# FFTAI/Wiki-GRx-Gym

Hardware: AMD Instinct MI355X
Metric: env-steps/sec GR1T1 rough-terrain @4096 envs (higher is better)
Workload: dtype f32

## Files before the change

include/grx_ppo.h:

```cpp
#ifndef GRX_PPO_H
#define GRX_PPO_H
#ifdef __cplusplus
extern "C" {
#endif

int grx_ppo_loss_partials_size(int batch);

int grx_ppo_loss(int batch, int num_actions, const float* mu, const float* std, const float* value,
                 const float* actions, const float* old_logp, const float* old_mu, const float* old_sigma,
                 const float* advantages, const float* returns, const float* target_values,
                 float clip_param, float value_loss_coef, float entropy_coef, int use_clipped_value_loss,
                 float* out, float* d_mu, float* d_std, float* d_value, float* partials, void* stream);

int grx_ppo_colsum_partials_size(int rows, int cols);
int grx_ppo_colsum(int rows, int cols, const float* x, float* out, float* partials, void* stream);

int grx_ppo_elu_backward_colsum(int rows, int cols, const float* dy, const float* y, float* dz, float* out, float* partials, void* stream);

int grx_ppo_store_transition(int N, int num_obs, int num_pri, int num_actions,
                             const float* obs, const float* pri, const float* actions, const float* mu, const float* sigma,
                             const float* values, const float* logp, const float* rewards, const unsigned char* dones,
                             const unsigned char* time_outs, float gamma,
                             float* st_obs, float* st_pri, float* st_actions, float* st_mu, float* st_sigma, float* st_values,
                             float* st_logp, float* st_rewards, unsigned char* st_dones,
// ... 2 lines not shown
#define GRX_PPO_TAIL_MAX 24
typedef struct grx_ppo_tail_tensors {
    int n, pad;
    float* param[GRX_PPO_TAIL_MAX]; const float* grad[GRX_PPO_TAIL_MAX]; float* exp_avg[GRX_PPO_TAIL_MAX]; float* exp_avg_sq[GRX_PPO_TAIL_MAX];
    float* step[GRX_PPO_TAIL_MAX];
    long long numel[GRX_PPO_TAIL_MAX];
} grx_ppo_tail_tensors;
typedef struct grx_ppo_tail_args {
    const float* loss;
    const float* bad_flag;
    const float* kl;
    float* lr;
    const float *value_loss, *surrogate_loss;
    float* sums;
    float* partials;
    int adaptive, pad;
    float desired_kl, lr_min, lr_max, max_grad_norm;
    double beta1, beta2, eps;
} grx_ppo_tail_args;
int grx_ppo_step_tail_blocks(const grx_ppo_tail_tensors* t);
int grx_ppo_step_tail(const grx_ppo_tail_tensors* t, const grx_ppo_tail_args* a, void* stream);

#define GRX_PPO_GATHER_MAX 12
int grx_ppo_gather_rows(int n_tensors, const float* const* src, float* const* dst, const int* widths, const long long* idx, int mb, void* stream);

int grx_mlp_layer(int M, int K, int N, const float* X, const float* W, const float* bias, float* Y, int elu, void* stream);

int grx_mlp_layer_bf16(int M, int K, int N, const float* X, const float* W, const float* bias, float* Y, int elu, void* stream);
int grx_mlp_input_grad_bf16(int M, int N, int K, const float* dZ, const float* W, float* dX, void* stream);
int grx_mlp_weight_grad_bf16_partials_size(int M, int N, int K);
int grx_mlp_weight_grad_bf16(int M, int N, int K, const float* dZ, const float* X, float* dW, float* partials, void* stream);

int grx_mlp_policy_head(int M, int K, int A, const float* X, const float* W, const float* bias, const float* std,
                        const float* eps, float* actions, float* logp, float* mu, float* sigma, void* stream);

int grx_obs_norm_partials_size(int rows, int cols);
int grx_obs_norm_moments(int rows, int cols, const float* x, float* partials, void* stream);
int grx_obs_norm_merge(int n_partials, int cols, int stride, const float* partials, long long* count, float* mean, float* var, float* std,
                       void* stream);
int grx_obs_norm_combine(int n_partials, int cols, const float* partials, float* out, void* stream);
int grx_obs_norm_apply(int rows, int cols, const float* x, const float* mean, const float* std, float eps, float* y, void* stream);
int grx_obs_norm_step(int rows, int cols, const float* x, float* partials, long long* count, float* mean, float* var, float* std, float eps,
                      float* y, void* stream);

int grx_obs_history_push(int N, int D, int H, const float* obs, const unsigned char* dones, int fill_all, const float* src, float* dst,
                         void* stream);

int grx_distill_loss_partials_size(int batch, int A);
int grx_distill_loss(int batch, int A, const float* student_mu, const float* teacher_mu, int huber, float* out, float* d_mu, float* partials,
                     void* stream);
int grx_distill_store(int N, int D, int A, const float* obs, const float* labels, const float* rewards, const unsigned char* dones,
                      float* st_obs, float* st_labels, unsigned char* st_dones,
                      float* cur_rew, float* cur_len, float* done_rew, float* done_len, void* stream);

int grx_lstm_cell(int M, int D, int H, const float* x, const float* h_prev, const float* c_prev, const unsigned char* reset,
                  const float* W_ih, const float* W_hh, const float* b_ih, const float* b_hh, float* h, float* c, float* acts, void* stream);
int grx_lstm_cell_preact(int M, int D, int H, const float* x, const float* h_prev, const unsigned char* reset, const float* W_ih,
                         const float* W_hh, const float* b_ih, const float* b_hh, float* G, void* stream);
int grx_lstm_cell_backward(int M, int H, const float* dh, const float* dc_in, const float* acts, const float* c_prev,
                           const unsigned char* reset, float* dG, float* dc_prev, void* stream);

#define GRX_SYM_MAX_WIDTH 2048
int grx_sym_gather_rows(int n_tensors, const float* const* src, float* const* dst, const int* widths, const int* modes,
                        const int* const* perm, const float* const* scale, const float* const* offset, const long long* idx, int mb,
                        void* stream);

int grx_rnd_reward_partials_size(int N);
int grx_rnd_reward(int N, int E, const float* pred, const float* targ, float gamma, float weight, float eps, float* ret, long long* count,
                   float* mean, float* var, float* std, float* rewards, float* intrinsic, float* raw, float* partials, void* stream);

#ifdef __cplusplus
}
#endif

#include "grx_ppo_noise.h"
#include "grx_ppo_smooth.h"
#include "grx_ppo_est.h"
#include "grx_ppo_gae.h"
#include "grx_ppo_gp.h"
#include "grx_ppo_ln.h"
#include "grx_ppo_mc.h"
#include "grx_ppo_beta.h"
#include "grx_ppo_cenet.h"
#endif
```

wiki-grx-gym_amd/csrc/grx_ppo.hip:

```cpp
#include <hip/hip_runtime.h>
#include <stdint.h>
#include "../../include/grx_ppo.h"

namespace {
constexpr int MAXA = 32;
constexpr int NTHR = 256;
constexpr int NRED = 3 + MAXA;

__device__ inline float nmax(float a, float b) { return (a > b || a != a) ? a : b; }
__device__ inline float nmin(float a, float b) { return (a < b || a != a) ? a : b; }

__device__ inline double wave_sum(double v) {
#pragma unroll
    for (int o = 32; o > 0; o >>= 1) v += __shfl_down(v, o);
    return v;
}

template <int A>
__global__ __launch_bounds__(NTHR) void ppo_loss_kernel(int B, const float* __restrict__ mu, const float* __restrict__ stdp,
                                                         const float* __restrict__ value, const float* __restrict__ actions,
                                                         const float* __restrict__ old_logp, const float* __restrict__ old_mu,
                                                         const float* __restrict__ old_sigma, const float* __restrict__ adv_,
                                                         const float* __restrict__ ret_, const float* __restrict__ tv_,
                                                         float clip, float vcoef, int use_clipped,
// ... 21 lines not shown
        const float rc = nmin(nmax(ratio, lo), hi);
        const float s1 = -adv * ratio, s2 = -adv * rc;
        const float surr = nmax(s1, s2);
        const float w1 = s1 > s2 ? 1.f : (s1 == s2 ? 0.5f : 0.f), w2 = 1.f - w1;
        const float in_range = (ratio >= lo && ratio <= hi) ? 1.f : 0.f;
        const float g_ratio = -adv * (w1 + w2 * in_range);
        const float g_logp = g_ratio * ratio * invB;
#pragma unroll
        for (int k = 0; k < A; ++k) {
            const float s = sg[k], inv2 = 1.0f / (s * s);
            const float half = 0.5f * inv2;
            const float np = 0.f * (g_logp * (((df[k] * df[k] * half) * half) * 2.0f * (2.0f * s)) - g_logp / s);
            d_mu[(size_t)i * A + k] = g_logp * df[k] * inv2 + np;
            red[3 + k] = g_logp * (df[k] * df[k] * inv2 / s - 1.0f / s) + np;
        }
        const float v = value[i], ret = ret_[i];
        float vl, gv;
        if (use_clipped) {
            const float tv = tv_[i];
            const float dv = v - tv;
            const float vc = tv + nmin(nmax(dv, -clip), clip);
            const float l1 = (v - ret) * (v - ret), l2 = (vc - ret) * (vc - ret);
            vl = nmax(l1, l2);
            const float u1 = l1 > l2 ? 1.f : (l1 == l2 ? 0.5f : 0.f), u2 = 1.f - u1;
            const float vin = (dv >= -clip && dv <= clip) ? 1.f : 0.f;
            gv = u1 * 2.0f * (v - ret) + (vin != 0.f ? u2 * 2.0f * (vc - ret) : 0.f);
        } else {
            vl = (ret - v) * (ret - v);
            gv = -2.0f * (ret - v);
        }
        d_value[i] = vcoef * gv * invB;
        red[0] = surr; red[1] = vl; red[2] = kl;
    }
    __shared__ double s_red[NTHR / 64][3 + A];
    const int lane = threadIdx.x & 63, wv = threadIdx.x >> 6;
#pragma unroll
    for (int k = 0; k < 3 + A; ++k) {
        const double t = wave_sum((double)red[k]);
        if (lane == 0) s_red[wv][k] = t;
    }
    __syncthreads();
    if (threadIdx.x < 3 + A) {
        double t = 0.0;
#pragma unroll
        for (int w = 0; w < NTHR / 64; ++w) t += s_red[w][threadIdx.x];
        partials[(size_t)blockIdx.x * NRED + threadIdx.x] = t;
    }
}

__global__ __launch_bounds__(64) void ppo_loss_finalize(int B, int A, int nblk, const double* __restrict__ partials,
                                                         const float* __restrict__ stdp, float vcoef, float ecoef,
                                                         float* __restrict__ out, float* __restrict__ d_std) {
    const int k = threadIdx.x;
    double t = 0.0;
    constexpr int STAGE = 4096;
    __shared__ double s_p[STAGE];
    const bool staged = nblk * NRED <= STAGE;
    if (staged) {
        for (int i = k; i < nblk * NRED; i += 64) s_p[i] = partials[i];
        __syncthreads();
    }
    if (k < 3 + A)
        for (int b = 0; b < nblk; ++b) t += staged ? s_p[b * NRED + k] : partials[(size_t)b * NRED + k];
    __shared__ double s_t[64];
    s_t[k] = t;
    __syncthreads();
    if (k >= 3 && k < 3 + A) d_std[k - 3] = (float)t - ecoef / stdp[k - 3];
    if (k == 0) {
        const float surr = (float)(s_t[0] / (double)B), vl = (float)(s_t[1] / (double)B), klm = (float)(s_t[2] / (double)B);
        float ent = 0.f;
        for (int a = 0; a < A; ++a) ent += 1.4189385332046727f + logf(stdp[a]);
        out[0] = surr; out[1] = vl; out[2] = surr + vcoef * vl - ecoef * ent; out[3] = klm;
    }
}

template <int A>
void launch(int nblk, hipStream_t st, int B, const float* mu, const float* stdp, const float* value, const float* actions,
            const float* old_logp, const float* old_mu, const float* old_sigma, const float* adv, const float* ret, const float* tv,
            float clip, float vcoef, int use_clipped, float* d_mu, float* d_value, double* partials) {
    hipLaunchKernelGGL(ppo_loss_kernel<A>, dim3(nblk), dim3(NTHR), 0, st, B, mu, stdp, value, actions, old_logp, old_mu, old_sigma,
                       adv, ret, tv, clip, vcoef, use_clipped, d_mu, d_value, partials);
}

constexpr int CS_ROWS = 256;
__global__ __launch_bounds__(256) void colsum_partial(int rows, int cols, const float* __restrict__ x, float* __restrict__ partials) {
    const int lane = threadIdx.x & 63, wv = threadIdx.x >> 6;
    const int col = blockIdx.x * 64 + lane;
    const int r0 = blockIdx.y * CS_ROWS, r1 = min(rows, r0 + CS_ROWS);
    float acc = 0.f;
    if (col < cols) {
        float a0 = 0.f, a1 = 0.f, a2 = 0.f, a3 = 0.f;
        int r = r0 + wv;
        for (; r + 12 < r1; r += 16) {
            a0 += x[(size_t)r * cols + col]; a1 += x[(size_t)(r + 4) * cols + col];
            a2 += x[(size_t)(r + 8) * cols + col]; a3 += x[(size_t)(r + 12) * cols + col];
        }
        for (; r < r1; r += 4) a0 += x[(size_t)r * cols + col];
        acc = (a0 + a1) + (a2 + a3);
    }
    __shared__ float s_acc[4][64];
    s_acc[wv][lane] = acc;
    __syncthreads();
    if (wv == 0 && col < cols) partials[(size_t)blockIdx.y * cols + col] = (s_acc[0][lane] + s_acc[1][lane]) + (s_acc[2][lane] + s_acc[3][lane]);
}
__global__ __launch_bounds__(256) void elu_bwd_colsum_partial(int rows, int cols, const float* __restrict__ dy, const float* __restrict__ y,
                                                              float* __restrict__ dz, float* __restrict__ partials) {
    const int lane = threadIdx.x & 63, wv = threadIdx.x >> 6;
    const int col = blockIdx.x * 64 + lane;
    const int r0 = blockIdx.y * CS_ROWS, r1 = min(rows, r0 + CS_ROWS);
    float acc = 0.f;
    if (col < cols) {
        float a0 = 0.f, a1 = 0.f, a2 = 0.f, a3 = 0.f;
        auto one = [&](const int r) -> float {
            const size_t o = (size_t)r * cols + col;
            const float yy = y[o];
            const float g = dy[o] * (yy > 0.f ? 1.0f : yy + 1.0f);
            dz[o] = g;
            return g;
        };
        int r = r0 + wv;
        for (; r + 12 < r1; r += 16) { a0 += one(r); a1 += one(r + 4); a2 += one(r + 8); a3 += one(r + 12); }
        for (; r < r1; r += 4) a0 += one(r);
        acc = (a0 + a1) + (a2 + a3);
    }
    __shared__ float s_acc[4][64];
    s_acc[wv][lane] = acc;
    __syncthreads();
    if (wv == 0 && col < cols) partials[(size_t)blockIdx.y * cols + col] = (s_acc[0][lane] + s_acc[1][lane]) + (s_acc[2][lane] + s_acc[3][lane]);
}
__global__ __launch_bounds__(256) void colsum_final(int cols, int nslab, const float* __restrict__ partials, float* __restrict__ out) {
    const int lane = threadIdx.x & 63, col = blockIdx.x * 4 + (threadIdx.x >> 6);
    if (col >= cols) return;
    float t = 0.f;
    for (int b = lane; b < nslab; b += 64) t += partials[(size_t)b * cols + col];
#pragma unroll
    for (int o = 32; o > 0; o >>= 1) t += __shfl_down(t, o);
    if (lane == 0) out[col] = t;
}

typedef float f32x16 __attribute__((ext_vector_type(16)));
constexpr int ML_BM = 64, ML_BN = 64, ML_KC = 64, ML_LD = 65;

__device__ inline float elu1(float x) { return x > 0.f ? x : expm1f(x); }

template <bool VEC>
__device__ inline void ml_fetch(const float* __restrict__ G, int rows, int ld, int r0, int k0, int tid, float4 v[4]) {
    const int kq = k0 + 4 * (tid & 15);
#pragma unroll
    for (int p = 0; p < 4; ++p) {
        const int r = r0 + 16 * p + (tid >> 4);
        const float* g = G + (size_t)min(r, rows - 1) * ld + kq;
        float4 x = {0.f, 0.f, 0.f, 0.f};
        if (r < rows) {
            if (VEC) { if (kq < ld) x = *reinterpret_cast<const float4*>(g); }
            else { if (kq < ld) x.x = g[0]; if (kq + 1 < ld) x.y = g[1]; if (kq + 2 < ld) x.z = g[2]; if (kq + 3 < ld) x.w = g[3]; }
        }
        v[p] = x;
    }
}
__device__ inline void ml_stash(float* __restrict__ S, int tid, const float4 v[4]) {
    const int kq = 4 * (tid & 15);
#pragma unroll
    for (int p = 0; p < 4; ++p) {
        float* s = S + kq * ML_LD + 16 * p + (tid >> 4);
        s[0] = v[p].x; s[ML_LD] = v[p].y; s[2 * ML_LD] = v[p].z; s[3 * ML_LD] = v[p].w;
    }
}

struct HeadOut { const float* stdp; const float* eps; float* actions; float* logp; float* mu; float* sigma; };
template <bool ELU, bool VEC, bool HEAD = false>
__global__ __launch_bounds__(256) void mlp_layer_kernel(int M, int K, int N, const float* __restrict__ X, const float* __restrict__ W,
                                                         const float* __restrict__ bias, float* __restrict__ Y, HeadOut ho = HeadOut()) {
#if defined(__HIP_DEVICE_COMPILE__) && !defined(__gfx950__)
#error "mlp_layer_kernel keeps 65 KB of static LDS: gfx950 (160 KB per CU) only -- this library is built for MI355X, see the Makefile"
#endif
    __shared__ float Xs[2][ML_KC * ML_LD], Ws[2][ML_KC * ML_LD];
    const int tid = threadIdx.x, lane = tid & 63, wv = tid >> 6, wy = wv >> 1, wx = wv & 1;
    const int m0 = blockIdx.x * ML_BM, n0 = blockIdx.y * ML_BN;
    float4 xr[4], wr[4];
    f32x16 acc;
#pragma unroll
    for (int r = 0; r < 16; ++r) acc[r] = 0.f;
    ml_fetch<VEC>(X, M, K, m0, 0, tid, xr);
    ml_fetch<VEC>(W, N, K, n0, 0, tid, wr);
    ml_stash(Xs[0], tid, xr); ml_stash(Ws[0], tid, wr);
    __syncthreads();
    int buf = 0;
    for (int k0 = 0; k0 < K; k0 += ML_KC, buf ^= 1) {
        const bool more = k0 + ML_KC < K;
        if (more) { ml_fetch<VEC>(X, M, K, m0, k0 + ML_KC, tid, xr); ml_fetch<VEC>(W, N, K, n0, k0 + ML_KC, tid, wr); }
        const float* xa = Xs[buf] + (lane >> 5) * ML_LD + 32 * wy + (lane & 31);
        const float* wb = Ws[buf] + (lane >> 5) * ML_LD + 32 * wx + (lane & 31);
        const int nk = min(ML_KC, K - k0);
        if (nk == ML_KC) {
            float av[ML_KC / 2], bv[ML_KC / 2];
#pragma unroll
            for (int kk = 0; kk < ML_KC / 2; ++kk) { av[kk] = xa[2 * kk * ML_LD]; bv[kk] = wb[2 * kk * ML_LD]; }
#pragma unroll
            for (int kk = 0; kk < ML_KC / 2; ++kk) acc = __builtin_amdgcn_mfma_f32_32x32x2f32(av[kk], bv[kk], acc, 0, 0, 0);
        } else {
            for (int kk = 0; kk < (nk + 1) / 2; ++kk)
                acc = __builtin_amdgcn_mfma_f32_32x32x2f32(xa[2 * kk * ML_LD], wb[2 * kk * ML_LD], acc, 0, 0, 0);
        }
        if (more) { ml_stash(Xs[buf ^ 1], tid, xr); ml_stash(Ws[buf ^ 1], tid, wr); }
        __syncthreads();
// ... 294 lines not shown
```

wiki-grx-gym_amd/rl/fused_loss.py:

```python
import ctypes as C
import os

import torch

_LIB = None


def load_ppo_library():
    global _LIB
    if _LIB is None:
        path = os.environ.get("GRX_PPO_LIB") or os.path.join(os.path.dirname(os.path.dirname(os.path.abspath(__file__))), "csrc", "libgrx_ppo.so")
        if not os.path.exists(path):
            raise RuntimeError(f"{path} is missing: build it with `python -c 'import __graft_entry__ as g; g.build()'` "
                               "(there is no silent fallback for CUDA tensors; set GRX_PPO_FUSED_LOSS=0 to use the torch expression)")
        lib = C.CDLL(path)
        fp = C.c_void_p
        lib.grx_ppo_loss.restype = C.c_int
        lib.grx_ppo_loss.argtypes = [C.c_int, C.c_int] + [fp] * 10 + [C.c_float, C.c_float, C.c_float, C.c_int] + [fp] * 5 + [C.c_void_p]
        lib.grx_ppo_loss_partials_size.restype = C.c_int
        lib.grx_ppo_loss_partials_size.argtypes = [C.c_int]
        lib.grx_ppo_colsum.restype = C.c_int
        lib.grx_ppo_colsum.argtypes = [C.c_int, C.c_int, fp, fp, fp, C.c_void_p]
        lib.grx_ppo_colsum_partials_size.restype = C.c_int
        lib.grx_ppo_colsum_partials_size.argtypes = [C.c_int, C.c_int]
# ... 3 lines not shown
        lib.grx_ppo_elu_backward_colsum.argtypes = [C.c_int, C.c_int, fp, fp, fp, fp, fp, C.c_void_p]
        lib.grx_ppo_gather_rows.restype = C.c_int
        lib.grx_ppo_gather_rows.argtypes = [C.c_int, C.POINTER(C.c_void_p), C.POINTER(C.c_void_p), C.POINTER(C.c_int), fp, C.c_int, C.c_void_p]
        lib.grx_mlp_layer.restype = C.c_int
        lib.grx_mlp_layer.argtypes = [C.c_int] * 3 + [fp] * 4 + [C.c_int, C.c_void_p]
        lib.grx_mlp_layer_bf16.restype = C.c_int
        lib.grx_mlp_layer_bf16.argtypes = [C.c_int] * 3 + [fp] * 4 + [C.c_int, C.c_void_p]
        lib.grx_mlp_input_grad_bf16.restype = C.c_int
        lib.grx_mlp_input_grad_bf16.argtypes = [C.c_int] * 3 + [fp] * 3 + [C.c_void_p]
        lib.grx_mlp_weight_grad_bf16_partials_size.restype = C.c_int
        lib.grx_mlp_weight_grad_bf16_partials_size.argtypes = [C.c_int] * 3
        lib.grx_mlp_weight_grad_bf16.restype = C.c_int
        lib.grx_mlp_weight_grad_bf16.argtypes = [C.c_int] * 3 + [fp] * 4 + [C.c_void_p]
        lib.grx_mlp_policy_head.restype = C.c_int
        lib.grx_mlp_policy_head.argtypes = [C.c_int] * 3 + [fp] * 9 + [C.c_void_p]
        lib.grx_ppo_step_tail.restype = C.c_int
        lib.grx_ppo_step_tail.argtypes = [C.c_void_p, C.c_void_p, C.c_void_p]
        lib.grx_ppo_step_tail_blocks.restype = C.c_int
        lib.grx_ppo_step_tail_blocks.argtypes = [C.c_void_p]
        lib.grx_obs_norm_partials_size.restype = C.c_int
        lib.grx_obs_norm_partials_size.argtypes = [C.c_int, C.c_int]
        lib.grx_obs_norm_moments.restype = C.c_int
        lib.grx_obs_norm_moments.argtypes = [C.c_int, C.c_int, fp, fp, C.c_void_p]
        lib.grx_obs_norm_merge.restype = C.c_int
        lib.grx_obs_norm_merge.argtypes = [C.c_int, C.c_int, C.c_int] + [fp] * 5 + [C.c_void_p]
        lib.grx_obs_norm_combine.restype = C.c_int
        lib.grx_obs_norm_combine.argtypes = [C.c_int, C.c_int, fp, fp, C.c_void_p]
        lib.grx_obs_norm_apply.restype = C.c_int
        lib.grx_obs_norm_apply.argtypes = [C.c_int, C.c_int, fp, fp, fp, C.c_float, fp, C.c_void_p]
        lib.grx_obs_norm_step.restype = C.c_int
        lib.grx_obs_norm_step.argtypes = [C.c_int, C.c_int] + [fp] * 6 + [C.c_float, fp, C.c_void_p]
        lib.grx_obs_history_push.restype = C.c_int
        lib.grx_obs_history_push.argtypes = [C.c_int] * 3 + [fp, fp, C.c_int, fp, fp, C.c_void_p]
        lib.grx_distill_loss_partials_size.restype = C.c_int
        lib.grx_distill_loss_partials_size.argtypes = [C.c_int, C.c_int]
        lib.grx_distill_loss.restype = C.c_int
        lib.grx_distill_loss.argtypes = [C.c_int, C.c_int, fp, fp, C.c_int, fp, fp, fp, C.c_void_p]
        lib.grx_distill_store.restype = C.c_int
        lib.grx_distill_store.argtypes = [C.c_int] * 3 + [fp] * 11 + [C.c_void_p]
        pp = C.POINTER(C.c_void_p)
        lib.grx_sym_gather_rows.restype = C.c_int
        lib.grx_sym_gather_rows.argtypes = [C.c_int, pp, pp, C.POINTER(C.c_int), C.POINTER(C.c_int), pp, pp, pp, fp, C.c_int, C.c_void_p]
        lib.grx_rnd_reward_partials_size.restype = C.c_int
        lib.grx_rnd_reward_partials_size.argtypes = [C.c_int]
        lib.grx_rnd_reward.restype = C.c_int
        lib.grx_rnd_reward.argtypes = [C.c_int, C.c_int, fp, fp, C.c_float, C.c_float, C.c_float] + [fp] * 9 + [C.c_void_p]
        lib.grx_ppo_loss_sd_partials_size.restype = C.c_int
        lib.grx_ppo_loss_sd_partials_size.argtypes = [C.c_int]
        lib.grx_ppo_loss_sd.restype = C.c_int
        lib.grx_ppo_loss_sd.argtypes = [C.c_int, C.c_int, fp, C.c_int] + [fp] * 8 + [C.c_float, C.c_float, C.c_float, C.c_int] + [fp] * 4 + [C.c_void_p]
        lib.grx_mlp_policy_head_sd.restype = C.c_int
        lib.grx_mlp_policy_head_sd.argtypes = [C.c_int] * 3 + [fp] * 3 + [C.c_int] + [fp] * 5 + [C.c_void_p]
        lib.grx_smooth_gather_rows.restype = C.c_int
        lib.grx_smooth_gather_rows.argtypes = ([C.c_int, pp, pp, C.POINTER(C.c_int), fp, C.c_int, C.c_int, C.c_int, fp, C.c_int, C.c_int, fp,
                                                C.c_float, fp, C.c_void_p])
        lib.grx_smooth_loss_partials_size.restype = C.c_int
        lib.grx_smooth_loss_partials_size.argtypes = [C.c_int, C.c_int]
        lib.grx_smooth_loss.restype = C.c_int
        lib.grx_smooth_loss.argtypes = [C.c_int, C.c_int, fp, C.c_int, C.c_int, fp, C.c_float, C.c_float, fp, fp, fp, C.c_void_p]
        lib.grx_est_forward.restype = C.c_int
        lib.grx_est_forward.argtypes = [fp, C.c_int, C.c_int, fp, C.c_int, fp, C.POINTER(C.c_int), fp, fp, C.c_void_p]
        lib.grx_gae_partials_size.restype = C.c_int
        lib.grx_gae_partials_size.argtypes = [C.c_int, C.c_int]
        lib.grx_gae_returns.restype = C.c_int
        lib.grx_gae_returns.argtypes = [C.c_int, C.c_int] + [fp] * 4 + [C.c_float] * 3 + [fp] * 10 + [C.c_void_p]
        lib.grx_gp_seed.restype = C.c_int
        lib.grx_gp_seed.argtypes = [C.c_int, C.c_int] + [fp] * 4 + [C.c_void_p]
        lib.grx_gp_gate.restype = C.c_int
        lib.grx_gp_gate.argtypes = [C.c_int, C.c_int] + [fp] * 3 + [C.c_void_p]
        lib.grx_gp_sqnorm_partials_size.restype = C.c_int
        lib.grx_gp_sqnorm_partials_size.argtypes = [C.c_int, C.c_int]
        lib.grx_gp_sqnorm.restype = C.c_int
        lib.grx_gp_sqnorm.argtypes = [C.c_int, C.c_int] + [fp] * 3 + [C.c_void_p]
        lib.grx_gp_gate_backward.restype = C.c_int
        lib.grx_gp_gate_backward.argtypes = [C.c_int, C.c_int] + [fp] * 8 + [C.c_void_p]
        lib.grx_gp_seed_backward.restype = C.c_int
        lib.grx_gp_seed_backward.argtypes = [C.c_int, C.c_int] + [fp] * 8 + [C.c_void_p]
        lib.grx_ln_elu_forward.restype = C.c_int
        lib.grx_ln_elu_forward.argtypes = [C.c_int, C.c_int, fp, fp, fp, C.c_float, fp, fp, fp, C.c_void_p]
        lib.grx_ln_elu_backward_partials_size.restype = C.c_int
        lib.grx_ln_elu_backward_partials_size.argtypes = [C.c_int, C.c_int]
        lib.grx_ln_elu_backward.restype = C.c_int
        lib.grx_ln_elu_backward.argtypes = [C.c_int, C.c_int] + [fp] * 11 + [C.c_void_p]
        _LIB = lib
    return _LIB


TAIL_MAX = 24


class _TailTensors(C.Structure):
    _fields_ = [("n", C.c_int), ("pad", C.c_int), ("param", C.c_void_p * TAIL_MAX), ("grad", C.c_void_p * TAIL_MAX),
                ("exp_avg", C.c_void_p * TAIL_MAX), ("exp_avg_sq", C.c_void_p * TAIL_MAX), ("step", C.c_void_p * TAIL_MAX),
                ("numel", C.c_longlong * TAIL_MAX)]


class _TailArgs(C.Structure):
    _fields_ = [("loss", C.c_void_p), ("bad_flag", C.c_void_p), ("kl", C.c_void_p), ("lr", C.c_void_p), ("value_loss", C.c_void_p),
                ("surrogate_loss", C.c_void_p), ("sums", C.c_void_p), ("partials", C.c_void_p), ("adaptive", C.c_int), ("pad", C.c_int),
                ("desired_kl", C.c_float), ("lr_min", C.c_float), ("lr_max", C.c_float), ("max_grad_norm", C.c_float),
                ("beta1", C.c_double), ("beta2", C.c_double), ("eps", C.c_double)]


class StepTail:

    @staticmethod
    def supported(optimizer, params):
        g = optimizer.param_groups
        return (len(g) == 1 and len(params) <= TAIL_MAX and not g[0].get("amsgrad") and not g[0].get("maximize") and g[0].get("weight_decay", 0) == 0
                and all(p.is_cuda and p.dtype == torch.float32 and p.is_contiguous() for p in params))

    def __init__(self, optimizer, params, lr_t):
        self.lib = load_ppo_library()
        self.opt, self.params, self.lr_t = optimizer, list(params), lr_t
        self.t, self.a = _TailTensors(), _TailArgs()
        self.key, self.partials = None, None

    def _state(self, p):
        st = self.opt.state[p]
        if "exp_avg" not in st:
            st["step"] = torch.zeros((), dtype=torch.float32, device=p.device)
            st["exp_avg"] = torch.zeros_like(p, memory_format=torch.preserve_format)
            st["exp_avg_sq"] = torch.zeros_like(p, memory_format=torch.preserve_format)
        return st

    def __call__(self, loss, kl, value_loss, surrogate_loss, sums, adaptive, desired_kl, lr_min, lr_max, max_grad_norm, bad_flag=None):
        t, a = self.t, self.a
        sts = [self._state(p) for p in self.params]
        key = tuple(x.data_ptr() for p, st in zip(self.params, sts) for x in (p, st["exp_avg"], st["exp_avg_sq"], st["step"]))
        if key != self.key:
            t.n = len(self.params)
            for i, (p, st) in enumerate(zip(self.params, sts)):
                if not (st["step"].is_cuda and st["step"].dtype == torch.float32 and st["exp_avg"].is_contiguous() and st["exp_avg_sq"].is_contiguous()):
                    raise RuntimeError("StepTail: the optimizer state is not torch's fused / capturable layout")
                t.param[i], t.exp_avg[i], t.exp_avg_sq[i], t.step[i], t.numel[i] = p.data_ptr(), st["exp_avg"].data_ptr(), st["exp_avg_sq"].data_ptr(), st["step"].data_ptr(), p.numel()
            nb = self.lib.grx_ppo_step_tail_blocks(C.byref(t))
            if nb < 1:
                raise RuntimeError("grx_ppo_step_tail_blocks failed")
            self.partials = torch.empty(nb, device=self.params[0].device, dtype=torch.float32)
            self.key = key
        for i, p in enumerate(self.params):
            g = p.grad
            if g is None or not g.is_contiguous() or g.dtype != torch.float32:
                raise RuntimeError("StepTail: every parameter needs a contiguous fp32 .grad")
            t.grad[i] = g.data_ptr()
        g0 = self.opt.param_groups[0]
        a.loss, a.kl, a.lr = loss.data_ptr(), kl.data_ptr(), self.lr_t.data_ptr()
        a.bad_flag = bad_flag.data_ptr() if bad_flag is not None else None
        a.value_loss, a.surrogate_loss = value_loss.data_ptr(), surrogate_loss.data_ptr()
        a.sums = sums.data_ptr() if sums is not None else None
        a.partials = self.partials.data_ptr()
        a.adaptive = int(bool(adaptive))
        a.desired_kl, a.lr_min, a.lr_max, a.max_grad_norm = float(desired_kl or 0.0), float(lr_min), float(lr_max), float(max_grad_norm)
        a.beta1, a.beta2, a.eps = float(g0["betas"][0]), float(g0["betas"][1]), float(g0["eps"])
        dev = self.params[0].device
        with torch.cuda.device(dev):
            rc = self.lib.grx_ppo_step_tail(C.byref(t), C.byref(a), C.c_void_p(torch.cuda.current_stream(dev).cuda_stream))
        if rc != 0:
            raise RuntimeError(f"grx_ppo_step_tail failed ({rc})")


def _f32c(x):
    return x if (x.dtype == torch.float32 and x.is_contiguous()) else x.contiguous().float()


class FusedPPOLoss(torch.autograd.Function):
# ... 22 lines not shown
        return out

    @staticmethod
    def backward(ctx, g):
        d_mu, d_std, d_value = ctx.saved_tensors
        gl = g[2]
        return (d_mu * gl, d_std * gl, (d_value * gl).reshape(ctx.value_shape)) + (None,) * 11


def fused_ppo_loss(mu, std, value, actions, old_logp, old_mu, old_sigma, advantages, returns, target_values,
                   clip_param, value_loss_coef, entropy_coef, use_clipped_value_loss):
    return FusedPPOLoss.apply(mu, std, value, actions, old_logp, old_mu, old_sigma, advantages, returns, target_values,
                              clip_param, value_loss_coef, entropy_coef, use_clipped_value_loss)


class FusedPPOLossSD(torch.autograd.Function):

    @staticmethod
    def forward(ctx, raw, value, actions, old_logp, old_mu, old_sigma, advantages, returns, target_values,
                log_std, clip_param, value_loss_coef, entropy_coef, use_clipped_value_loss):
        lib = load_ppo_library()
        B, A = actions.shape
        if tuple(raw.shape) != (B, 2 * A):
            raise RuntimeError(f"fused_ppo_loss_sd: raw is {tuple(raw.shape)}, expected {(B, 2 * A)} ([mean | s] of {A} actions)")
        raw_c, value_c = _f32c(raw), _f32c(value).reshape(-1)
        data = [_f32c(t) for t in (actions, old_logp, old_mu, old_sigma, advantages, returns, target_values)]
        out = torch.empty(4, device=raw.device, dtype=torch.float32)
        d_raw = torch.empty_like(raw_c)
        d_value = torch.empty_like(value_c)
        partials = torch.empty(lib.grx_ppo_loss_sd_partials_size(B), device=raw.device, dtype=torch.float32)
        stream = torch.cuda.current_stream(raw.device).cuda_stream
        with torch.cuda.device(raw.device):
            rc = lib.grx_ppo_loss_sd(B, A, raw_c.data_ptr(), int(bool(log_std)), value_c.data_ptr(), *[t.data_ptr() for t in data],
                                     float(clip_param), float(value_loss_coef), float(entropy_coef), int(bool(use_clipped_value_loss)),
                                     out.data_ptr(), d_raw.data_ptr(), d_value.data_ptr(), partials.data_ptr(), C.c_void_p(stream))
        if rc != 0:
            raise RuntimeError(f"grx_ppo_loss_sd failed ({rc}): batch {B}, num_actions {A}")
        ctx.save_for_backward(d_raw, d_value)
        ctx.value_shape = value.shape
        return out

    @staticmethod
    def backward(ctx, g):
        d_raw, d_value = ctx.saved_tensors
        gl = g[2]
        return (d_raw * gl, (d_value * gl).reshape(ctx.value_shape)) + (None,) * 12


def fused_ppo_loss_sd(raw, value, actions, old_logp, old_mu, old_sigma, advantages, returns, target_values,
                      log_std, clip_param, value_loss_coef, entropy_coef, use_clipped_value_loss):
    return FusedPPOLossSD.apply(raw, value, actions, old_logp, old_mu, old_sigma, advantages, returns, target_values,
                                log_std, clip_param, value_loss_coef, entropy_coef, use_clipped_value_loss)


def colsum(x):
    lib = load_ppo_library()
    x = _f32c(x)
    rows, cols = x.shape
    out = torch.empty(cols, device=x.device, dtype=torch.float32)
    partials = torch.empty(lib.grx_ppo_colsum_partials_size(rows, cols), device=x.device, dtype=torch.float32)
    with torch.cuda.device(x.device):
        rc = lib.grx_ppo_colsum(rows, cols, x.data_ptr(), out.data_ptr(), partials.data_ptr(),
                                C.c_void_p(torch.cuda.current_stream(x.device).cuda_stream))
    if rc != 0:
        raise RuntimeError(f"grx_ppo_colsum failed ({rc}): {rows} x {cols}")
    return out


def elu_backward_colsum(dy, y):
    lib = load_ppo_library()
    dy, y = _f32c(dy), _f32c(y)
    rows, cols = dy.shape
    dz = torch.empty_like(dy)
    out = torch.empty(cols, device=dy.device, dtype=torch.float32)
    partials = torch.empty(lib.grx_ppo_colsum_partials_size(rows, cols), device=dy.device, dtype=torch.float32)
    with torch.cuda.device(dy.device):
        rc = lib.grx_ppo_elu_backward_colsum(rows, cols, dy.data_ptr(), y.data_ptr(), dz.data_ptr(), out.data_ptr(), partials.data_ptr(),
                                             C.c_void_p(torch.cuda.current_stream(dy.device).cuda_stream))
    if rc != 0:
        raise RuntimeError(f"grx_ppo_elu_backward_colsum failed ({rc}): {rows} x {cols}")
    return dz, out


def store_transition(storage, step, obs, pri, actions, mu, sigma, values, logp, rewards, dones, time_outs, gamma, log=None):
    lib = load_ppo_library()
    N = storage.num_envs
    ptr = lambda t: t.data_ptr() if t is not None else None
    for t in (obs, pri, actions, mu, sigma, values, logp, rewards):
        if t is not None and not (t.is_cuda and t.dtype == torch.float32 and t.is_contiguous()):
            raise RuntimeError("store_transition needs contiguous float32 CUDA tensors")
    def as_u8(t):
        if t.dtype == torch.bool:
            t = t.view(torch.uint8)
        elif t.dtype != torch.uint8:
            t = (t != 0).to(torch.uint8)
        if not (t.is_cuda and t.is_contiguous() and t.numel() == N):
            raise RuntimeError("store_transition needs contiguous CUDA dones / time_outs with one entry per env")
        return t
    d8 = as_u8(dones)
    t8 = None if time_outs is None else as_u8(time_outs)
    sp = storage.pri_observations
    lg = log if log is not None else (None, None, None, None)
    with torch.cuda.device(obs.device):
        rc = lib.grx_ppo_store_transition(
            N, obs.shape[1], pri.shape[1] if (pri is not None and sp is not None) else 0, actions.shape[1],
            ptr(obs), ptr(pri) if sp is not None else None, ptr(actions), ptr(mu), ptr(sigma), ptr(values), ptr(logp), ptr(rewards), ptr(d8), ptr(t8),
            float(gamma), ptr(storage.observations[step]), ptr(sp[step]) if sp is not None else None, ptr(storage.actions[step]), ptr(storage.mu[step]),
            ptr(storage.sigma[step]), ptr(storage.values[step]), ptr(storage.actions_log_prob[step]), ptr(storage.rewards[step]), ptr(storage.dones[step]),
            ptr(lg[0]), ptr(lg[1]), ptr(lg[2]), ptr(lg[3]), C.c_void_p(torch.cuda.current_stream(obs.device).cuda_stream))
    if rc != 0:
        raise RuntimeError(f"grx_ppo_store_transition failed ({rc})")


def _linears_of(mlp):
    mods = list(mlp.model)
    lin = []
    for i, m in enumerate(mods):
        if i % 2 == 0:
            if not isinstance(m, torch.nn.Linear):
                return None
            lin.append((m.weight, m.bias))
        elif not (isinstance(m, torch.nn.ELU) and m.alpha == 1.0):
            return None
    return lin if len(mods) % 2 == 1 else None


LN_MAX_COLS = 1024


def ln_fused():
    return os.environ.get("GRX_LN_FUSED", "1") != "0"


def _layers_of(mlp):
    mods = list(mlp.model)
    layers, i = [], 0
    while i < len(mods):
        m = mods[i]
        if not isinstance(m, torch.nn.Linear):
            return None
        if i + 1 == len(mods):
            layers.append((m.weight, m.bias, None))
            return layers
        norm = None
        if isinstance(mods[i + 1], torch.nn.LayerNorm):
            norm = mods[i + 1]
            if not (norm.elementwise_affine and norm.bias is not None and tuple(norm.normalized_shape) == (m.out_features,)
                    and m.out_features <= LN_MAX_COLS):
                return None
            i += 1
        if not (i + 1 < len(mods) and isinstance(mods[i + 1], torch.nn.ELU) and mods[i + 1].alpha == 1.0):
            return None
        layers.append((m.weight, m.bias, norm))
        i += 2
    return None


def mlp_can_fuse(mlp, x):
    if not (x.is_cuda and x.dtype == torch.float32 and x.dim() == 2):
        return False
    layers = _layers_of(mlp)
    return layers is not None and (ln_fused() or all(n is None for _, _, n in layers))


def ln_elu_forward(z, gamma, beta, eps, stats=True):
    lib = load_ppo_library()
# ... 208 lines not shown
```

wiki-grx-gym_amd/rl/modules.py:

```python
import torch
import torch.nn as nn
from torch.distributions import Normal

PRECISIONS = ("fp32", "bf16")
_ACTIVATIONS = {"elu": nn.ELU, "selu": nn.SELU, "relu": nn.ReLU, "crelu": nn.ReLU, "lrelu": nn.LeakyReLU,
                "tanh": nn.Tanh, "sigmoid": nn.Sigmoid}


def get_activation(name):
    if name not in _ACTIVATIONS:
        print("invalid activation function!")
        return None
    return _ACTIVATIONS[name]()


import os

_FUSED_ELU_FORWARD = os.environ.get("GRX_PPO_FUSED_FWD", "1") != "0"
_FUSED_ELU_BACKWARD = os.environ.get("GRX_PPO_FUSED_ELU", "1") != "0"
_TRAIN_LINEAR = os.environ.get("GRX_PPO_LINEAR", "colsum")


class _TrainLinear(torch.autograd.Function):

    @staticmethod
    def _blas(pin):
        prev = torch.backends.cuda.preferred_blas_library()
        if pin:
            torch.backends.cuda.preferred_blas_library("cublaslt")
        return prev

    @staticmethod
    def forward(ctx, x, weight, bias):
        prev = _TrainLinear._blas(weight.shape[0] == 1)
        try:
            y = torch.addmm(bias, x, weight.t())
        finally:
            torch.backends.cuda.preferred_blas_library(prev)
        ctx.save_for_backward(x, weight)
        return y

    @staticmethod
    def backward(ctx, dy):
        from .fused_loss import colsum
        x, weight = ctx.saved_tensors
        prev = _TrainLinear._blas(weight.shape[0] == 1)
        try:
            dx = dy @ weight if ctx.needs_input_grad[0] else None
            return dx, dy.t() @ x, colsum(dy)
        finally:
            torch.backends.cuda.preferred_blas_library(prev)


class _TrainLinearELU(torch.autograd.Function):

    @staticmethod
    def forward(ctx, x, weight, bias, bf16):
        ctx.bf16 = bf16
        if bf16:
            from .fused_loss import linear_elu
            y = linear_elu(x, weight, bias, bf16=True)
        elif _FUSED_ELU_FORWARD and x.is_contiguous() and weight.is_contiguous():
            from .fused_loss import linear_elu
            y = linear_elu(x, weight, bias)
        else:
            prev = _TrainLinear._blas(weight.shape[0] == 1)
            try:
                y = torch.nn.functional.elu(torch.addmm(bias, x, weight.t()))
            finally:
                torch.backends.cuda.preferred_blas_library(prev)
        ctx.save_for_backward(x, weight, y)
        return y

    @staticmethod
    def backward(ctx, dy):
        from .fused_loss import elu_backward_colsum
        x, weight, y = ctx.saved_tensors
        dz, db = elu_backward_colsum(dy, y)
        if ctx.bf16:
            from .fused_loss import input_grad_bf16, weight_grad_bf16
            dx = input_grad_bf16(dz, weight) if ctx.needs_input_grad[0] else None
            return dx, weight_grad_bf16(dz, x), db, None
        prev = _TrainLinear._blas(weight.shape[0] == 1)
        try:
            dx = dz @ weight if ctx.needs_input_grad[0] else None
            return dx, dz.t() @ x, db, None
        finally:
            torch.backends.cuda.preferred_blas_library(prev)


def ln_elu_torch(x, weight, bias, gamma, beta, eps):
    z = torch.addmm(bias, x, weight.t())
    return torch.nn.functional.elu(torch.nn.functional.layer_norm(z, (z.shape[-1],), gamma, beta, eps)), z


def ln_elu_backward_torch(dy, y, z, gamma, eps):
    m = z.mean(-1, keepdim=True)
    d = z - m
    s = 1.0 / torch.sqrt((d * d).mean(-1, keepdim=True) + eps)
    xh = d * s
    g = dy * torch.where(y > 0, torch.ones_like(y), y + 1.0)
    q = g * gamma
    c1, c2 = q.mean(-1, keepdim=True), (q * xh).mean(-1, keepdim=True)
    dz = s * ((q - c1) - xh * c2)
    return dz, (g * xh).sum(0), g.sum(0), dz.sum(0)


class _TrainLinearLNELU(torch.autograd.Function):

    @staticmethod
    def forward(ctx, x, weight, bias, gamma, beta, eps):
        from .fused_loss import ln_fused
        ctx.eps, ctx.fused = float(eps), bool(x.is_cuda and ln_fused())
        if ctx.fused:
            from .fused_loss import _f32c, _layer, ln_elu_forward, load_ppo_library
            with torch.cuda.device(x.device):
                z = _layer(load_ppo_library(), _f32c(x), _f32c(weight), bias, False, torch.cuda.current_stream(x.device).cuda_stream)
            y, mean, rstd = ln_elu_forward(z, gamma, beta, ctx.eps)
            ctx.save_for_backward(x, weight, gamma, z, y, mean, rstd)
            return y
        prev = _TrainLinear._blas(x.is_cuda and weight.shape[0] == 1)
        try:
            y, z = ln_elu_torch(x, weight, bias, gamma, beta, ctx.eps)
        finally:
            torch.backends.cuda.preferred_blas_library(prev)
        ctx.save_for_backward(x, weight, gamma, z, y)
        return y

    @staticmethod
    def backward(ctx, dy):
        if ctx.fused:
            from .fused_loss import ln_elu_backward
            x, weight, gamma, z, y, mean, rstd = ctx.saved_tensors
            dz, dgamma, dbeta, db = ln_elu_backward(dy, y, z, mean, rstd, gamma)
        else:
            x, weight, gamma, z, y = ctx.saved_tensors
            dz, dgamma, dbeta, db = ln_elu_backward_torch(dy, y, z, gamma, ctx.eps)
        prev = _TrainLinear._blas(x.is_cuda and weight.shape[0] == 1)
        try:
            dx = dz @ weight if ctx.needs_input_grad[0] else None
            return dx, dz.t() @ x, db, dgamma, dbeta, None
        finally:
            torch.backends.cuda.preferred_blas_library(prev)


class MLP(nn.Module):
    def __init__(self, input_size, output_size, hidden_dims=(256, 256, 256), activation="relu", layer_norm=False, layer_norm_eps=1e-5, **_):
        super().__init__()
        self.input_size, self.output_size, self.hidden_dims = input_size, output_size, list(hidden_dims)
        self.layer_norm, self.layer_norm_eps = bool(layer_norm), float(layer_norm_eps)
        if self.layer_norm and activation != "elu":
            raise ValueError(f"MLP: layer_norm=True needs activation='elu' (the fused LayerNorm + ELU pass), not {activation!r}")
        if self.layer_norm and not self.layer_norm_eps > 0.0:
            raise ValueError(f"MLP: layer_norm_eps must be above 0, not {layer_norm_eps!r}")
        if self.layer_norm and any(not 1 <= int(h) <= 1024 for h in hidden_dims):
            raise ValueError(f"MLP: layer_norm=True covers hidden widths of 1..1024 (include/grx_ppo_ln.h), not {list(hidden_dims)}")
        dims = [input_size] + list(hidden_dims)
        layers = []
        for a, b in zip(dims[:-1], dims[1:]):
            if self.layer_norm:
# ... 273 lines not shown
```

Measured before the change: 97.81 million.

## Add fused f32 MFMA hidden-layer backward computing dX and split-K dW in one kernel

Adds a hidden-layer backward path for fp32 ELU layers. It runs the ELU-grad column sum, then one persistent MFMA kernel that computes both the input gradient and split-K partial weight gradients from a shared work list, then a finish kernel that reduces the dW and bias partials. It replaces separate BLAS GEMMs plus the colsum, and is enabled only for shape/batch ranges listed in a hand-tuned table. The kernel is gfx950-only and needs an extra partials buffer allocation on every call.

```diff
diff --git a/include/grx_ppo.h b/include/grx_ppo.h
--- a/include/grx_ppo.h
+++ b/include/grx_ppo.h
@@ -108,4 +108,5 @@
 #include "grx_ppo_mc.h"
 #include "grx_ppo_beta.h"
 #include "grx_ppo_cenet.h"
+#include "grx_ppo_bwd.h"
 #endif
diff --git a/include/grx_ppo_bwd.h b/include/grx_ppo_bwd.h
--- /dev/null
+++ b/include/grx_ppo_bwd.h
@@ -0,0 +1,20 @@
+#ifndef GRX_PPO_BWD_H
+#define GRX_PPO_BWD_H
+#ifdef __cplusplus
+extern "C" {
+#endif
+
+int grx_mlp_hidden_backward_f32_partials_size(int M, int N, int K);
+
+int grx_mlp_hidden_backward_f32(int M, int N, int K,
+                                const float* dY, const float* Y,
+                                const float* X, const float* W,
+                                float* dZ,
+                                float* dX,
+                                float* dW, float* db,
+                                float* partials, void* stream);
+
+#ifdef __cplusplus
+}
+#endif
+#endif
diff --git a/wiki-grx-gym_amd/csrc/grx_ppo.hip b/wiki-grx-gym_amd/csrc/grx_ppo.hip
--- a/wiki-grx-gym_amd/csrc/grx_ppo.hip
+++ b/wiki-grx-gym_amd/csrc/grx_ppo.hip
@@ -127,7 +127,7 @@
                        adv, ret, tv, clip, vcoef, use_clipped, d_mu, d_value, partials);
 }
 
-constexpr int CS_ROWS = 256;
+#include "grx_ppo_colsum.h"
 __global__ __launch_bounds__(256) void colsum_partial(int rows, int cols, const float* __restrict__ x, float* __restrict__ partials) {
     const int lane = threadIdx.x & 63, wv = threadIdx.x >> 6;
     const int col = blockIdx.x * 64 + lane;
@@ -141,31 +141,6 @@
             a2 += x[(size_t)(r + 8) * cols + col]; a3 += x[(size_t)(r + 12) * cols + col];
         }
         for (; r < r1; r += 4) a0 += x[(size_t)r * cols + col];
-        acc = (a0 + a1) + (a2 + a3);
-    }
-    __shared__ float s_acc[4][64];
-    s_acc[wv][lane] = acc;
-    __syncthreads();
-    if (wv == 0 && col < cols) partials[(size_t)blockIdx.y * cols + col] = (s_acc[0][lane] + s_acc[1][lane]) + (s_acc[2][lane] + s_acc[3][lane]);
-}
-__global__ __launch_bounds__(256) void elu_bwd_colsum_partial(int rows, int cols, const float* __restrict__ dy, const float* __restrict__ y,
-                                                              float* __restrict__ dz, float* __restrict__ partials) {
-    const int lane = threadIdx.x & 63, wv = threadIdx.x >> 6;
-    const int col = blockIdx.x * 64 + lane;
-    const int r0 = blockIdx.y * CS_ROWS, r1 = min(rows, r0 + CS_ROWS);
-    float acc = 0.f;
-    if (col < cols) {
-        float a0 = 0.f, a1 = 0.f, a2 = 0.f, a3 = 0.f;
-        auto one = [&](const int r) -> float {
-            const size_t o = (size_t)r * cols + col;
-            const float yy = y[o];
-            const float g = dy[o] * (yy > 0.f ? 1.0f : yy + 1.0f);
-            dz[o] = g;
-            return g;
-        };
-        int r = r0 + wv;
-        for (; r + 12 < r1; r += 16) { a0 += one(r); a1 += one(r + 4); a2 += one(r + 8); a3 += one(r + 12); }
-        for (; r < r1; r += 4) a0 += one(r);
         acc = (a0 + a1) + (a2 + a3);
     }
     __shared__ float s_acc[4][64];
diff --git a/wiki-grx-gym_amd/csrc/grx_ppo_bwd.hip b/wiki-grx-gym_amd/csrc/grx_ppo_bwd.hip
--- /dev/null
+++ b/wiki-grx-gym_amd/csrc/grx_ppo_bwd.hip
@@ -0,0 +1,231 @@
+#include <hip/hip_runtime.h>
+#include <stdint.h>
+#include "../../include/grx_ppo.h"
+
+namespace {
+#include "grx_ppo_colsum.h"
+
+typedef float f32x16 __attribute__((ext_vector_type(16)));
+constexpr int PT = 128, PKC = 32, PLD = PT + 4, NT = 256;
+constexpr int SLOTS = 512;
+constexpr int MIN_SLAB = 128;
+
+struct Plan {
+    int M, N, K;
+    int tkx, ndx;
+    int tkw, tw, slab, nslab;
+    int nitems;
+};
+
+inline int cdiv(int a, int b) { return (a + b - 1) / b; }
+
+inline Plan make_plan(int M, int N, int K, bool dx) {
+    Plan p;
+    p.M = M; p.N = N; p.K = K;
+    p.tkx = cdiv(K, PT);
+    p.ndx = dx ? cdiv(M, PT) * p.tkx : 0;
+    p.tkw = cdiv(K, PT);
+    p.tw = cdiv(N, PT) * p.tkw;
+    int slab = cdiv(N, PKC) * PKC;
+    if (slab > 512) slab = 512;
+    while (slab > MIN_SLAB && (long long)cdiv(M, slab) * p.tw < 2 * SLOTS) slab = cdiv(slab / 2, PKC) * PKC;
+    if (slab < MIN_SLAB) slab = MIN_SLAB;
+    p.slab = slab;
+    p.nslab = cdiv(M, slab);
+    p.nitems = p.ndx + p.nslab * p.tw;
+    return p;
+}
+
+struct Walk { int a, step, b, lim_a, lim_b; };
+template <bool VEC>
+__device__ inline void fetch(const float* __restrict__ G, int ld, const Walk w, float4 v[4]) {
+#pragma unroll
+    for (int p = 0; p < 4; ++p) {
+        const float* g = G + (size_t)min(w.a + w.step * p, w.lim_a - 1) * ld;
+        if (VEC) v[p] = *reinterpret_cast<const float4*>(g + min(w.b, w.lim_b - 4));
+        else { const int e = w.lim_b - 1; v[p].x = g[min(w.b, e)]; v[p].y = g[min(w.b + 1, e)]; v[p].z = g[min(w.b + 2, e)]; v[p].w = g[min(w.b + 3, e)]; }
+    }
+}
+template <bool VEC>
+__device__ inline void mask(const Walk w, float4 v[4]) {
+#pragma unroll
+    for (int p = 0; p < 4; ++p) {
+        const bool in_a = w.a + w.step * p < w.lim_a;
+        const bool o0 = in_a && w.b < w.lim_b, o1 = VEC ? o0 : (in_a && w.b + 1 < w.lim_b), o2 = VEC ? o0 : (in_a && w.b + 2 < w.lim_b),
+                   o3 = VEC ? o0 : (in_a && w.b + 3 < w.lim_b);
+        v[p].x = o0 ? v[p].x : 0.f; v[p].y = o1 ? v[p].y : 0.f; v[p].z = o2 ? v[p].z : 0.f; v[p].w = o3 ? v[p].w : 0.f;
+    }
+}
+__device__ inline void stash_rowc(float* __restrict__ S, int tid, const float4 v[4]) {
+#pragma unroll
+    for (int p = 0; p < 4; ++p) *reinterpret_cast<float4*>(S + ((tid >> 5) + 8 * p) * PLD + 4 * (tid & 31)) = v[p];
+}
+__device__ inline void stash_kc(float* __restrict__ S, int tid, const float4 v[4]) {
+#pragma unroll
+    for (int p = 0; p < 4; ++p) {
+        float* s = S + 4 * (tid & 7) * PLD + (tid >> 3) + 32 * p;
+        s[0] = v[p].x; s[PLD] = v[p].y; s[2 * PLD] = v[p].z; s[3 * PLD] = v[p].w;
+    }
+}
+
+__device__ inline int xcd_order(int q, int n) {
+    const int fl = n >> 3, big = n & 7, x = q & 7;
+    return (x < big ? x * (fl + 1) : big * (fl + 1) + (x - big) * fl) + (q >> 3);
+}
+
+template <bool VN, bool VK>
+__global__ __launch_bounds__(NT, 2) void pair_kernel(const Plan P, const float* __restrict__ dZ, const float* __restrict__ X,
+                                                     const float* __restrict__ W, float* __restrict__ dX, float* __restrict__ pw) {
+#if defined(__HIP_DEVICE_COMPILE__) && !defined(__gfx950__)
+#error "pair_kernel keeps 66 KB of static LDS and uses v_mfma_f32_32x32x2_f32: gfx950 only -- this library is built for MI355X, see the Makefile"
+#endif
+    __shared__ float As[2][PKC * PLD], Bs[2][PKC * PLD];
+    const int tid = threadIdx.x, lane = tid & 63, wv = tid >> 6, wy = wv >> 1, wx = wv & 1;
+    const int M = P.M, N = P.N, K = P.K;
+    for (int item = blockIdx.x; item < P.nitems; item += gridDim.x) {
+        const bool isx = item < P.ndx;
+        int r0, c0, kb, ke, rowsD;
+        float* D;
+        if (isx) {
+            const int li = xcd_order(item, P.ndx), mt = li / P.tkx;
+            r0 = mt * PT; c0 = (li - mt * P.tkx) * PT; kb = 0; ke = N; D = dX; rowsD = M;
+        } else {
+            const int j = xcd_order(item - P.ndx, P.nitems - P.ndx), s = j / P.tw, t = j - s * P.tw, nt = t / P.tkw;
+            r0 = nt * PT; c0 = (t - nt * P.tkw) * PT; kb = s * P.slab; ke = min(M, kb + P.slab); D = pw + (size_t)s * N * K; rowsD = N;
+        }
+        const float* Bg = isx ? W : X;
+        f32x16 acc[2][2];
+#pragma unroll
+        for (int i = 0; i < 2; ++i)
+#pragma unroll
+            for (int j = 0; j < 2; ++j)
+#pragma unroll
+                for (int r = 0; r < 16; ++r) acc[i][j][r] = 0.f;
+        Walk wa = isx ? Walk{r0 + (tid >> 3), 32, kb + 4 * (tid & 7), M, ke} : Walk{kb + (tid >> 5), 8, r0 + 4 * (tid & 31), ke, N};
+        Walk wb = Walk{kb + (tid >> 5), 8, c0 + 4 * (tid & 31), ke, K};
+        const int da = isx ? 0 : PKC, db = isx ? PKC : 0;
+        float4 ar[4], br[4];
+        fetch<VN>(dZ, N, wa, ar);
+        fetch<VK>(Bg, K, wb, br);
+        mask<VN>(wa, ar); mask<VK>(wb, br);
+        if (isx) stash_kc(As[0], tid, ar); else stash_rowc(As[0], tid, ar);
+        stash_rowc(Bs[0], tid, br);
+        __syncthreads();
+        int buf = 0;
+        for (int k0 = kb; k0 < ke; k0 += PKC, buf ^= 1) {
+            const bool more = k0 + PKC < ke;
+            if (more) {
+                wa.a += da; wa.b += db; wb.a += PKC;
+                fetch<VN>(dZ, N, wa, ar);
+                fetch<VK>(Bg, K, wb, br);
+            }
+            const float* xa = As[buf] + (lane >> 5) * PLD + 64 * wy + (lane & 31);
+            const float* xb = Bs[buf] + (lane >> 5) * PLD + 64 * wx + (lane & 31);
+            float a0[3], a1[3], b0[3], b1[3];
+            a0[0] = xa[0]; a1[0] = xa[32]; b0[0] = xb[0]; b1[0] = xb[32];
+            a0[1] = xa[2 * PLD]; a1[1] = xa[2 * PLD + 32]; b0[1] = xb[2 * PLD]; b1[1] = xb[2 * PLD + 32];
+#pragma unroll
+            for (int kk = 0; kk < PKC / 2; ++kk) {
+                const int cur = kk % 3, n = (kk + 2) % 3;
+                if (kk + 2 < PKC / 2) {
+                    const int o = 2 * (kk + 2) * PLD;
+                    a0[n] = xa[o]; a1[n] = xa[o + 32]; b0[n] = xb[o]; b1[n] = xb[o + 32];
+                }
+                acc[0][0] = __builtin_amdgcn_mfma_f32_32x32x2f32(a0[cur], b0[cur], acc[0][0], 0, 0, 0);
+                acc[0][1] = __builtin_amdgcn_mfma_f32_32x32x2f32(a0[cur], b1[cur], acc[0][1], 0, 0, 0);
+                acc[1][0] = __builtin_amdgcn_mfma_f32_32x32x2f32(a1[cur], b0[cur], acc[1][0], 0, 0, 0);
+                acc[1][1] = __builtin_amdgcn_mfma_f32_32x32x2f32(a1[cur], b1[cur], acc[1][1], 0, 0, 0);
+                __builtin_amdgcn_sched_group_barrier(0x100, 2, 0);
+                __builtin_amdgcn_sched_group_barrier(0x008, 4, 0);
+            }
+            if (more) {
+                mask<VN>(wa, ar); mask<VK>(wb, br);
+                if (isx) stash_kc(As[buf ^ 1], tid, ar); else stash_rowc(As[buf ^ 1], tid, ar);
+                stash_rowc(Bs[buf ^ 1], tid, br);
+            }
+            __syncthreads();
+        }
+#pragma unroll
+        for (int j = 0; j < 2; ++j) {
+            const int col = c0 + 64 * wx + 32 * j + (lane & 31);
+            if (col >= K) continue;
+#pragma unroll
+            for (int i = 0; i < 2; ++i)
+#pragma unroll
+                for (int r = 0; r < 16; ++r) {
+                    const int row = r0 + 64 * wy + 32 * i + (r & 3) + 8 * (r >> 2) + 4 * (lane >> 5);
+                    if (row < rowsD) D[(size_t)row * K + col] = acc[i][j][r];
+                }
+        }
+    }
+}
+
+__global__ __launch_bounds__(256) void finish_kernel(int n, int nslab, const float* __restrict__ pw, float* __restrict__ dW, int nbw,
+                                                     int cols, int ncs, const float* __restrict__ pc, float* __restrict__ db) {
+    if ((int)blockIdx.x < nbw) {
+        const int i = blockIdx.x * 256 + threadIdx.x;
+        if (i >= n) return;
+        float t = 0.f;
+        int s = 0;
+        for (; s + 16 <= nslab; s += 16) {
+            float v[16];
+#pragma unroll
+            for (int j = 0; j < 16; ++j) v[j] = pw[(size_t)(s + j) * n + i];
+#pragma unroll
+            for (int j = 0; j < 16; ++j) t += v[j];
+        }
+        for (; s < nslab; ++s) t += pw[(size_t)s * n + i];
+        dW[i] = t;
+        return;
+    }
+    const int lane = threadIdx.x & 63, col = (blockIdx.x - nbw) * 4 + (threadIdx.x >> 6);
+    if (col >= cols) return;
+    float t = 0.f;
+    for (int b = lane; b < ncs; b += 64) t += pc[(size_t)b * cols + col];
+#pragma unroll
+    for (int o = 32; o > 0; o >>= 1) t += __shfl_down(t, o);
+    if (lane == 0) db[col] = t;
+}
+
+inline bool al16(const void* p) { return ((uintptr_t)p & 15) == 0; }
+
+inline int resident_slots() {
+    static int slots[64] = {0};
+    int dev = 0;
+    if (hipGetDevice(&dev) != hipSuccess || dev < 0 || dev >= 64) return SLOTS;
+    if (slots[dev] == 0) {
+        int cus = 0;
+        slots[dev] = (hipDeviceGetAttribute(&cus, hipDeviceAttributeMultiprocessorCount, dev) == hipSuccess && cus > 0) ? 2 * cus : SLOTS;
+    }
+    return slots[dev];
+}
+}
+
+extern "C" int grx_mlp_hidden_backward_f32_partials_size(int M, int N, int K) {
+    if (M < 1 || N < 1 || K < 1) return 0;
+    const Plan p = make_plan(M, N, K, false);
+    const long long n = (long long)cdiv(M, CS_ROWS) * N + (long long)p.nslab * N * K;
+    return n > 0x7fffffffLL ? 0 : (int)n;
+}
+
+extern "C" int grx_mlp_hidden_backward_f32(int M, int N, int K, const float* dY, const float* Y, const float* X, const float* W,
+                                           float* dZ, float* dX, float* dW, float* db, float* partials, void* stream) {
+    if (M < 1 || N < 1 || K < 1 || !dY || !Y || !X || !W || !dZ || !dW || !db || !partials) return -1;
+    if (grx_mlp_hidden_backward_f32_partials_size(M, N, K) < 1) return -1;
+    hipStream_t st = (hipStream_t)stream;
+    const Plan p = make_plan(M, N, K, dX != nullptr);
+    const int ncs = cdiv(M, CS_ROWS);
+    float* pc = partials;
+    float* pw = partials + (size_t)ncs * N;
+    hipLaunchKernelGGL(elu_bwd_colsum_partial, dim3(cdiv(N, 64), ncs), dim3(256), 0, st, M, N, dY, Y, dZ, pc);
+    const int slots = resident_slots();
+    const bool vn = N % 4 == 0 && al16(dZ), vk = K % 4 == 0 && al16(X) && al16(W);
+    const dim3 grid(p.nitems < slots ? p.nitems : slots);
+#define GRX_PAIR_LAUNCH(VN, VK) hipLaunchKernelGGL((pair_kernel<VN, VK>), grid, dim3(NT), 0, st, p, (const float*)dZ, X, W, dX, pw)
+    if (vn) { if (vk) GRX_PAIR_LAUNCH(true, true); else GRX_PAIR_LAUNCH(true, false); }
+    else { if (vk) GRX_PAIR_LAUNCH(false, true); else GRX_PAIR_LAUNCH(false, false); }
+#undef GRX_PAIR_LAUNCH
+    const int n = N * K, nbw = cdiv(n, 256);
+    hipLaunchKernelGGL(finish_kernel, dim3(nbw + cdiv(N, 4)), dim3(256), 0, st, n, p.nslab, (const float*)pw, dW, nbw, N, ncs, (const float*)pc, db);
+    return hipGetLastError() == hipSuccess ? 0 : -2;
+}
diff --git a/wiki-grx-gym_amd/csrc/grx_ppo_colsum.h b/wiki-grx-gym_amd/csrc/grx_ppo_colsum.h
--- /dev/null
+++ b/wiki-grx-gym_amd/csrc/grx_ppo_colsum.h
@@ -0,0 +1,29 @@
+#ifndef GRX_PPO_COLSUM_H
+#define GRX_PPO_COLSUM_H
+constexpr int CS_ROWS = 256;
+__global__ __launch_bounds__(256) void elu_bwd_colsum_partial(int rows, int cols, const float* __restrict__ dy, const float* __restrict__ y,
+                                                              float* __restrict__ dz, float* __restrict__ partials) {
+    const int lane = threadIdx.x & 63, wv = threadIdx.x >> 6;
+    const int col = blockIdx.x * 64 + lane;
+    const int r0 = blockIdx.y * CS_ROWS, r1 = min(rows, r0 + CS_ROWS);
+    float acc = 0.f;
+    if (col < cols) {
+        float a0 = 0.f, a1 = 0.f, a2 = 0.f, a3 = 0.f;
+        auto one = [&](const int r) -> float {
+            const size_t o = (size_t)r * cols + col;
+            const float yy = y[o];
+            const float g = dy[o] * (yy > 0.f ? 1.0f : yy + 1.0f);
+            dz[o] = g;
+            return g;
+        };
+        int r = r0 + wv;
+        for (; r + 12 < r1; r += 16) { a0 += one(r); a1 += one(r + 4); a2 += one(r + 8); a3 += one(r + 12); }
+        for (; r < r1; r += 4) a0 += one(r);
+        acc = (a0 + a1) + (a2 + a3);
+    }
+    __shared__ float s_acc[4][64];
+    s_acc[wv][lane] = acc;
+    __syncthreads();
+    if (wv == 0 && col < cols) partials[(size_t)blockIdx.y * cols + col] = (s_acc[0][lane] + s_acc[1][lane]) + (s_acc[2][lane] + s_acc[3][lane]);
+}
+#endif
diff --git a/wiki-grx-gym_amd/rl/fused_loss.py b/wiki-grx-gym_amd/rl/fused_loss.py
--- a/wiki-grx-gym_amd/rl/fused_loss.py
+++ b/wiki-grx-gym_amd/rl/fused_loss.py
@@ -109,6 +109,10 @@
         lib.grx_ln_elu_backward_partials_size.argtypes = [C.c_int, C.c_int]
         lib.grx_ln_elu_backward.restype = C.c_int
         lib.grx_ln_elu_backward.argtypes = [C.c_int, C.c_int] + [fp] * 11 + [C.c_void_p]
+        lib.grx_mlp_hidden_backward_f32_partials_size.restype = C.c_int
+        lib.grx_mlp_hidden_backward_f32_partials_size.argtypes = [C.c_int] * 3
+        lib.grx_mlp_hidden_backward_f32.restype = C.c_int
+        lib.grx_mlp_hidden_backward_f32.argtypes = [C.c_int] * 3 + [fp] * 9 + [C.c_void_p]
         _LIB = lib
     return _LIB
 
@@ -297,6 +301,27 @@
     return dz, out
 
 
+def hidden_backward_f32(dy, y, x, w, need_dx):
+    lib = load_ppo_library()
+    dy, y, x, w = _f32c(dy), _f32c(y), _f32c(x), _f32c(w)
+    (M, N), K = dy.shape, w.shape[1]
+    size = lib.grx_mlp_hidden_backward_f32_partials_size(M, N, K)
+    if size < 1:
+        raise RuntimeError(f"grx_mlp_hidden_backward_f32 refuses the shape {M} x {N} x {K}")
+    dz = torch.empty_like(dy)
+    dx = torch.empty(M, K, device=dy.device, dtype=torch.float32) if need_dx else None
+    dw = torch.empty(N, K, device=dy.device, dtype=torch.float32)
+    db = torch.empty(N, device=dy.device, dtype=torch.float32)
+    partials = torch.empty(size, device=dy.device, dtype=torch.float32)
+    with torch.cuda.device(dy.device):
+        rc = lib.grx_mlp_hidden_backward_f32(M, N, K, dy.data_ptr(), y.data_ptr(), x.data_ptr(), w.data_ptr(), dz.data_ptr(),
+                                             dx.data_ptr() if need_dx else None, dw.data_ptr(), db.data_ptr(), partials.data_ptr(),
+                                             C.c_void_p(torch.cuda.current_stream(dy.device).cuda_stream))
+    if rc != 0:
+        raise RuntimeError(f"grx_mlp_hidden_backward_f32 failed ({rc}): {M} x {N} x {K}")
+    return dx, dw, db
+
+
 def store_transition(storage, step, obs, pri, actions, mu, sigma, values, logp, rewards, dones, time_outs, gamma, log=None):
     lib = load_ppo_library()
     N = storage.num_envs
diff --git a/wiki-grx-gym_amd/rl/modules.py b/wiki-grx-gym_amd/rl/modules.py
--- a/wiki-grx-gym_amd/rl/modules.py
+++ b/wiki-grx-gym_amd/rl/modules.py
@@ -19,6 +19,17 @@
 _FUSED_ELU_FORWARD = os.environ.get("GRX_PPO_FUSED_FWD", "1") != "0"
 _FUSED_ELU_BACKWARD = os.environ.get("GRX_PPO_FUSED_ELU", "1") != "0"
 _TRAIN_LINEAR = os.environ.get("GRX_PPO_LINEAR", "colsum")
+_BWD_F32 = os.environ.get("GRX_PPO_BWD", "pair") != "blas"
+
+
+_BWD_F32_WINS = {(128, 256, True): (2048, 24576), (256, 512, True): (10485, 24576),
+                 (512, 39, False): (24576, 24576), (512, 105, False): (24576, 24576), (512, 168, False): (24576, 24576),
+                 (512, 234, False): (24576, 24576)}
+
+
+def _bwd_f32_pick(M, N, K, need_dx):
+    lo, hi = _BWD_F32_WINS.get((N, K, bool(need_dx)), (1, 0))
+    return lo <= M <= hi
 
 
 class _TrainLinear(torch.autograd.Function):
@@ -76,6 +87,11 @@
     def backward(ctx, dy):
         from .fused_loss import elu_backward_colsum
         x, weight, y = ctx.saved_tensors
+        if not ctx.bf16 and _BWD_F32 and dy.dim() == 2 and all(t.is_cuda and t.dtype == torch.float32 and t.is_contiguous() for t in (dy, y, x, weight)) \
+                and _bwd_f32_pick(dy.shape[0], weight.shape[0], weight.shape[1], ctx.needs_input_grad[0]):
+            from .fused_loss import hidden_backward_f32
+            dx, dw, db = hidden_backward_f32(dy, y, x, weight, ctx.needs_input_grad[0])
+            return dx, dw, db, None
         dz, db = elu_backward_colsum(dy, y)
         if ctx.bf16:
             from .fused_loss import input_grad_bf16, weight_grad_bf16
```

Result: no change. 97.81 million (-0.0%).
